# daultanigaurav/AI-BASED-FRAME-INTERPOLATION

Hardware: AMD Instinct MI355X
Metric: interpolated frames/sec at 1080p (higher is better)
Workload: dtype bf16

## Files before the change

ai_based_frame_interpolation_amd/csrc/conv3x3_kwave.hip.h:

```cpp
#pragma once
#include "conv3x3_mfma.hip.h"

namespace fiunet {

struct KWaveTile {
    static constexpr int BN = 64, TH = 2, TW = 32;
    static constexpr int TWP = 40, THP = TH + 2;
    static constexpr int IN_BYTES = THP * TWP * 64;
    static constexpr int W_BYTES = 3 * BN * 64;
    static constexpr int W_SLOTS = 2;
    static constexpr int WAVE_BYTES = IN_BYTES + W_SLOTS * W_BYTES;
    static constexpr int LDS_BYTES = 4 * WAVE_BYTES;
    static_assert(LDS_BYTES <= 160 * 1024, "one workgroup per CU: 160 KiB of LDS");
    static_assert(16 * 1024 <= WAVE_BYTES, "a wave's partial sums (16 KiB) are exchanged through its own region");
};

template <int EPI, bool X2 = false, typename T = __bf16>
__global__ __launch_bounds__(256, 1) void conv3x3_kwave_kernel(const ConvArgs a)
{
    using Tile = KWaveTile;
    constexpr int PL = Elem<T>::PL;
    static_assert(!X2 || std::is_same_v<T, __bf16>, "two-piece operands are bf16");
    constexpr int TWP = Tile::TWP, THP = Tile::THP, TW = Tile::TW, TH = Tile::TH, BN = Tile::BN;
    constexpr int FR = 2, NF = 4, ROWS_W = 2;
    static_assert(EPI == EPI_PLAIN || EPI == EPI_POOL, "plain or pooled epilogue");
    static_assert(conv_wave_frags(64, 8, 32) == NF, "the epilogue is instantiated for the 64 x 64 wave tile");

    extern __shared__ __attribute__((aligned(16))) char smem[];
    const int tid = threadIdx.x;
    const int lane = tid & 63, wave = __builtin_amdgcn_readfirstlane(tid >> 6);
    const int l15 = lane & 15, lc = lane >> 4;
    char* const my = smem + wave * Tile::WAVE_BYTES;
    char* const lds_in = my;
    char* const lds_w = my + Tile::IN_BYTES;
    const unsigned lds_in_addr = lds_addr_of(lds_in);
    const unsigned lds_w_addr = lds_addr_of(lds_w);

    const ConvTileId id = conv_tile_decode(a, conv_block_remap());
    const int ct = id.ct, b = id.b;
    const int y0 = id.ty * TH, x0 = id.tx * TW;
    const int aH = a.H, aW = a.W;

    const int nplanes = (a.C0 + a.C1) / PL;
    const int p0 = a.C0 / PL;
    const int pbeg = wave * nplanes / 4, pend = (wave + 1) * nplanes / 4;
    constexpr int VP = X2 ? 3 : 1;
    const int nsteps = (pend - pbeg) * 3 * VP;
    f32x4 acc[4][NF];
#pragma unroll
    for (int m = 0; m < 4; ++m) {
        f32x4 v = f32x4{0.f, 0.f, 0.f, 0.f};
        if (wave == 0) {
            const float4 sh = *reinterpret_cast<const float4*>(a.shift + ct * BN + conv_cout_ofs<T>(m, lc));
            v = f32x4{sh.x, sh.y, sh.z, sh.w};
        }
#pragma unroll
        for (int n = 0; n < NF; ++n) acc[m][n] = v;
    }

    const int a_off = l15 * 64 + ((lc ^ swz(l15)) << 4);
    int b_off[3];
#pragma unroll
    for (int kx = 0; kx < 3; ++kx) b_off[kx] = (kx + l15) * 64 + ((lc ^ swz(kx + l15)) << 4);

    const char* const wbase = (const char*)a.wgt + (size_t)ct * BN * 64;
    const unsigned w_lane_off = (unsigned)((lane >> 2) * 64 + (((lane & 3) ^ swz(lane >> 2)) << 4));
    constexpr int NWP = Tile::W_BYTES / 1024;
    auto issue_w = [&](int step) __attribute__((always_inline)) {
        const int lp = step / 3, kx = step - lp * 3;
        int pl = pbeg + lp;
        if constexpr (X2) {
            const int real = pbeg + lp / 3;
            pl = lp % 3 == 1 ? nplanes + real : real;
        }
        const char* wsrc = wbase + ((size_t)(pl * 9 + kx * 3) * a.Cout) * 64;
        const unsigned dst = __builtin_amdgcn_readfirstlane(lds_w_addr + (unsigned)((step & 1) * Tile::W_BYTES));
#pragma unroll
        for (int j = 0; j < NWP; ++j) {
            const int r0 = j * 16, tap = r0 / BN;
            glds16s(wsrc + (size_t)(tap * (a.Cout - BN) + r0) * 64, w_lane_off, dst + j * 1024);
        }
    };
    if (nsteps > 0) issue_w(0);

    constexpr int NPIECE = THP * TWP / 16;
    static_assert(THP * TWP % 16 == 0, "in-tile must be a whole number of 1-KiB pieces");
    const char* const dma_src = (const char*)a.src0 + (size_t)b * aH * aW * a.C0 * sizeof(T) * (X2 ? 2 : 1);
    const char* const dma_src1 = a.C1 > 0 ? (const char*)a.src1 + (size_t)b * aH * aW * a.C1 * sizeof(T) * (X2 ? 2 : 1) : nullptr;
    const unsigned plane_bytes = (unsigned)(aH * aW) * 64u;
    unsigned in_off[NPIECE];
#pragma unroll
    for (int j = 0; j < NPIECE; ++j) {
        const int row = j * 16 + (lane >> 2);
        const int py = row / TWP, px = row - py * TWP;
        const int y = y0 - 1 + py, x = x0 - 1 + px;
        const bool ok = (px < TW + 2) & ((unsigned)y < (unsigned)aH) & ((unsigned)x < (unsigned)aW);
        in_off[j] = ok ? (unsigned)(y * aW + x) * 64u + (((lane & 3) ^ swz(row)) << 4) : ~0u;
        if (!ok) *reinterpret_cast<uint4*>(lds_in + j * 1024 + lane * 16) = make_uint4(0u, 0u, 0u, 0u);
    }
    auto gather_plane = [&](int plane, bool lo) __attribute__((always_inline)) {
        const char* base = plane >= p0 ? dma_src1 + (size_t)(plane - p0 + (lo ? nplanes - p0 : 0)) * plane_bytes
                                       : dma_src + (size_t)(plane + (lo ? p0 : 0)) * plane_bytes;
#pragma unroll
        for (int j = 0; j < NPIECE; ++j)
            if (in_off[j] != ~0u) glds16s(base, in_off[j], __builtin_amdgcn_readfirstlane(lds_in_addr + (unsigned)j * 1024u));
    };
    if (nsteps > 0) gather_plane(pbeg, false);
    lds_dma_wait_all();

    int step = 0;
    const int nvp = (pend - pbeg) * VP;
    for (int vp = 0; vp < nvp; ++vp) {
        const int nreal = pbeg + (vp + 1) / VP, nj = (vp + 1) % VP;
        const bool gather_next = vp + 1 < nvp && !(X2 && nj == 1);
#pragma unroll
        for (int kx = 0; kx < 3; ++kx, ++step) {
            if (step + 1 < nsteps) issue_w(step + 1);
            const char* wcur = lds_w + (step & 1) * Tile::W_BYTES + a_off;
            const bool next_tile = kx == 2 && gather_next;
            uint4 xb[ROWS_W + 2][FR];
            auto load_row = [&](int i) __attribute__((always_inline)) {
#pragma unroll
                for (int f = 0; f < FR; ++f)
                    xb[i][f] = *reinterpret_cast<const uint4*>(lds_in + b_off[kx] + (i * TWP + f * 16) * 64);
            };
#pragma unroll
            for (int i = 0; i < ROWS_W; ++i) load_row(i);
#pragma unroll
            for (int ky = 0; ky < 3; ++ky) {
                uint4 wa[4];
#pragma unroll
                for (int m = 0; m < 4; ++m) wa[m] = *reinterpret_cast<const uint4*>(wcur + (ky * BN + m * 16) * 64);
                if (ky < 2) load_row(ROWS_W + ky);
                if (ky == 1 && next_tile) {
                    asm volatile("s_waitcnt lgkmcnt(0)" ::: "memory");
                    gather_plane(nreal, X2 && nj == 2);
                }
#pragma unroll
                for (int m = 0; m < 4; ++m)
#pragma unroll
                    for (int n = 0; n < NF; ++n) mma_chunk<T>(acc[m][n], wa[m], xb[n / FR + ky][n % FR]);
            }
            lds_dma_wait_all();
        }
    }

    if (wave != 0) {
        float4* o = reinterpret_cast<float4*>(my) + lane;
#pragma unroll
        for (int m = 0; m < 4; ++m)
#pragma unroll
            for (int n = 0; n < NF; ++n)
                o[(m * NF + n) * 64] = make_float4(acc[m][n][0], acc[m][n][1], acc[m][n][2], acc[m][n][3]);
    }
    __syncthreads();
    if (wave != 0) return;
#pragma unroll
    for (int w = 1; w < 4; ++w) {
        const float4* p = reinterpret_cast<const float4*>(smem + w * Tile::WAVE_BYTES) + lane;
#pragma unroll
        for (int m = 0; m < 4; ++m)
#pragma unroll
            for (int n = 0; n < NF; ++n) {
                const float4 q = p[(m * NF + n) * 64];
                acc[m][n][0] += q.x; acc[m][n][1] += q.y; acc[m][n][2] += q.z; acc[m][n][3] += q.w;
            }
    }
    conv_epilogue<T, 64, 8, 32, EPI, X2>(a, acc, b, y0, x0, ct, 0, 0, 0, l15, lc);
}

}
```

ai_based_frame_interpolation_amd/csrc/conv3x3_mfma.hip.h:

```cpp
#pragma once
#include <hip/hip_runtime.h>
#include <stdint.h>
#include <type_traits>

namespace fiunet {

typedef __attribute__((ext_vector_type(4))) float f32x4;
typedef __attribute__((ext_vector_type(8))) __bf16 bf16x8;
typedef __attribute__((ext_vector_type(8))) _Float16 f16x8;

enum SrcMode { SRC_DIRECT = 0, SRC_POOL = 1 , SRC_CONCAT_UP = 2,
               SRC_STEM = 3 ,
               SRC_DIRECT_X2 = 4,
               SRC_STEM_X2 = 5 };
constexpr bool src_is_stem(int mode) { return mode == SRC_STEM || mode == SRC_STEM_X2; }
constexpr bool src_is_x2(int mode) { return mode == SRC_DIRECT_X2 || mode == SRC_STEM_X2; }

__device__ __forceinline__ size_t blk_off(int plane, int y, int x, int H, int W)
{
    return (((size_t)plane * H + y) * W + x) * 64;
}

struct ConvArgs {
    const void* src0;
// ... 411 lines not shown
}

template <typename T, int BN, int TH, int TW, int EPI>
__device__ __forceinline__ void conv_acc_init(const ConvArgs& a, f32x4 (&acc)[4][conv_wave_frags(BN, TH, TW)],
                                              int ct, int wc, int lc)
{
    constexpr int NF = conv_wave_frags(BN, TH, TW);
#pragma unroll
    for (int m = 0; m < 4; ++m) {
        f32x4 v = f32x4{0.f, 0.f, 0.f, 0.f};
        if constexpr (!epi_is_splitk(EPI)) {
            const float4 sh = *reinterpret_cast<const float4*>(a.shift + ct * BN + wc * 64 + conv_cout_ofs<T>(m, lc));
            v = f32x4{sh.x, sh.y, sh.z, sh.w};
        }
#pragma unroll
        for (int n = 0; n < NF; ++n) acc[m][n] = v;
    }
}

__device__ __forceinline__ unsigned relu_pk_bf16(unsigned p) { return pk_max_i16(p, 0u); }
__device__ __forceinline__ void relu_fma(float& sum, float x, float lo, float w)
{
    float t;
    asm("v_max_f32 %1, %3, %2\n\tv_fmac_f32 %0, %1, %4" : "+v"(sum), "=&v"(t) : "v"(x), "v"(lo), "v"(w));
}

template <typename T, int BN, int TH, int TW, int EPI, bool X2 = false>
__device__ __forceinline__ void conv_epilogue(const ConvArgs& a, f32x4 (&acc)[4][conv_wave_frags(BN, TH, TW)],
                                              int b, int y0, int x0, int ct, int split, int wc, int wp,
                                              int l15, int lc)
{
    constexpr int PL = Elem<T>::PL;
    constexpr int FR = TW / 16;
    constexpr int NF = conv_wave_frags(BN, TH, TW);
    constexpr int ROWS_W = NF / FR;
    constexpr int HNC = EPI == EPI_HEAD ? 1 : (EPI == EPI_HEAD3 ? 3 : 0);
    const int aH = a.H, aW = a.W;
    constexpr bool PERM = sizeof(T) == 2;
    const int wbase_c = ct * BN + wc * 64;
    if constexpr (epi_is_splitk(EPI)) {
        const int tile = (((b * a.tilesY) + y0 / TH) * a.tilesX + x0 / TW) * a.nct + ct;
        const int ntile = a.B * a.tilesY * a.tilesX * a.nct;
        const int wave = wp * (BN / 64) + wc;
        float4* o = reinterpret_cast<float4*>(a.kslab) + ((((size_t)split * ntile + tile) * 4 + wave) * (4 * NF)) * 64 + (lc * 16 + l15);
#pragma unroll
        for (int m = 0; m < 4; ++m)
#pragma unroll
            for (int n = 0; n < NF; ++n)
                o[(m * NF + n) * 64] = make_float4(acc[m][n][0], acc[m][n][1], acc[m][n][2], acc[m][n][3]);
        return;
    }
    float hw[HNC > 0 ? HNC : 1][4][4];
#pragma unroll
    for (int c = 0; c < HNC; ++c)
#pragma unroll
        for (int m = 0; m < 4; ++m) {
            const float4 v = *reinterpret_cast<const float4*>(a.head_w + c * 64 + conv_cout_ofs<T>(m, lc));
            hw[c][m][0] = v.x; hw[c][m][1] = v.y; hw[c][m][2] = v.z; hw[c][m][3] = v.w;
        }
    const size_t plane_stride = (size_t)aH * aW * 64;
    const int plane0 = wbase_c / PL;
    const int rec_byte = lc * 16;
    char* const out_img = a.dst ? (char*)a.dst + (size_t)b * plane_stride * (a.Cout / PL) +
                                  (size_t)plane0 * plane_stride + rec_byte : nullptr;
    const int pH = aH >> 1, pW = aW >> 1;
    const size_t pplane_stride = (size_t)pH * pW * 64;
    char* const pool_img = EPI == EPI_POOL ? (char*)a.pool_dst + (size_t)b * pplane_stride * (a.Cout / PL) +
                                             (size_t)plane0 * pplane_stride + rec_byte : nullptr;
    if constexpr (HNC > 0) {
        static_assert(HNC == 0 || NF == 8 || NF == 4, "head reduction is written for 8 or 4 fragments per wave");
        const float floor_v = a.relu ? 0.f : -__builtin_inff();
        float hb[HNC];
#pragma unroll
        for (int c = 0; c < HNC; ++c) hb[c] = a.head_b[c];
        const int nb = ((lc & 1) ? 4 : 0) + ((lc & 2) ? 2 : 0);
#pragma unroll
        for (int c = 0; c < HNC; ++c) {
            float hs[NF];
#pragma unroll
            for (int n = 0; n < NF; ++n) {
                float sum = 0.f;
#pragma unroll
                for (int m = 0; m < 4; ++m)
#pragma unroll
                    for (int j = 0; j < 4; ++j) relu_fma(sum, acc[m][n][j], floor_v, hw[c][m][j]);
                hs[n] = sum;
            }
            if constexpr (NF == 4) {
                float full[NF];
#pragma unroll
                for (int n = 0; n < NF; ++n) {
                    const float p = hs[n] + __shfl_xor(hs[n], 16);
                    full[n] = p + __shfl_xor(p, 32);
                }
                const float mine = lc == 0 ? full[0] : (lc == 1 ? full[1] : (lc == 2 ? full[2] : full[3]));
                const int n = lc;
                const int y = y0 + wp * ROWS_W + n / FR;
                const int x = x0 + (n % FR) * 16 + l15;
                if (y < aH && x < aW) {
                    const size_t o = (size_t)b * a.head_img_stride + ((size_t)c * aH + y) * aW + x;
                    if (a.head_out_u8) a.head_out_u8[o] = postprocess_u8_value(mine + hb[c]);
                    else a.head_out[o] = mine + hb[c];
                }
            } else {
                float t[4], u[2];
#pragma unroll
                for (int i = 0; i < 4; ++i) {
                    const auto r = __builtin_amdgcn_permlane16_swap(__float_as_uint(hs[i]), __float_as_uint(hs[(i + 4) % NF]), false, false);
                    t[i] = __uint_as_float(r[0]) + __uint_as_float(r[1]);
                }
#pragma unroll
                for (int j = 0; j < 2; ++j) {
                    const auto r = __builtin_amdgcn_permlane32_swap(__float_as_uint(t[j]), __float_as_uint(t[j + 2]), false, false);
                    u[j] = __uint_as_float(r[0]) + __uint_as_float(r[1]);
                }
#pragma unroll
                for (int j = 0; j < 2; ++j) {
                    const int n = nb + j;
                    const int y = y0 + wp * ROWS_W + n / FR;
                    const int x = x0 + (n % FR) * 16 + l15;
                    if (y < aH && x < aW) {
                        const size_t o = (size_t)b * a.head_img_stride + ((size_t)c * aH + y) * aW + x;
                        if (a.head_out_u8) a.head_out_u8[o] = postprocess_u8_value(u[j] + hb[c]);
                        else a.head_out[o] = u[j] + hb[c];
                    }
                }
            }
        }
    }
    if constexpr (X2) {
        static_assert(std::is_same_v<T, __bf16>, "the two-piece epilogue belongs to the bf16 kernels");
        if (HNC > 0 && !a.dst) return;
        const size_t ps = (size_t)aH * aW * 64;
        const int npo = a.Cout / 32;
        const size_t blk = (size_t)npo * ps;
        char* const img = (char*)a.dst + (size_t)b * 2 * blk + (size_t)(wbase_c / 32) * ps + lc * 16;
        const int pH2 = aH >> 1, pW2 = aW >> 1;
        const size_t pps = (size_t)pH2 * pW2 * 64, pblk = (size_t)npo * pps;
        char* const pimg = EPI == EPI_POOL ? (char*)a.pool_dst + (size_t)b * 2 * pblk + (size_t)(wbase_c / 32) * pps + lc * 16
                                           : nullptr;
        auto put = [&](char* o, size_t block_bytes, const float (&v)[8]) __attribute__((always_inline)) {
            unsigned h[4], l[4];
#pragma unroll
            for (int i = 0; i < 4; ++i) {
                h[i] = pack_bf16x2_pk(v[2 * i], v[2 * i + 1]);
                l[i] = pack_bf16x2_pk(v[2 * i] - __uint_as_float(h[i] << 16), v[2 * i + 1] - __uint_as_float(h[i] & 0xffff0000u));
            }
            *reinterpret_cast<uint4*>(o) = make_uint4(h[0], h[1], h[2], h[3]);
            *reinterpret_cast<uint4*>(o + block_bytes) = make_uint4(l[0], l[1], l[2], l[3]);
        };
#pragma unroll
        for (int n = 0; n < NF; ++n) {
            const int y = y0 + wp * ROWS_W + n / FR;
            const int x = x0 + (n % FR) * 16 + l15;
            if (y < aH && x < aW) {
#pragma unroll
                for (int g = 0; g < 2; ++g) {
                    float v[8];
#pragma unroll
                    for (int j = 0; j < 4; ++j) {
                        v[j] = a.relu ? fmaxf(acc[2 * g][n][j], 0.f) : acc[2 * g][n][j];
                        v[4 + j] = a.relu ? fmaxf(acc[2 * g + 1][n][j], 0.f) : acc[2 * g + 1][n][j];
                    }
                    put(img + (size_t)(y * aW + x) * 64 + g * ps, blk, v);
                }
            }
        }
        if constexpr (EPI == EPI_POOL) {
#pragma unroll
            for (int n = 0; n < NF; ++n) {
                if (((n / FR) & 1) != 0) continue;
                const int y = y0 + wp * ROWS_W + n / FR;
                const int x = x0 + (n % FR) * 16 + l15;
                const int py = y >> 1, px = x >> 1;
                const bool okp = (py < pH2) && (px < pW2) && ((l15 & 1) == 0);
#pragma unroll
                for (int g = 0; g < 2; ++g) {
                    float v[8];
#pragma unroll
                    for (int h = 0; h < 2; ++h)
#pragma unroll
                        for (int j = 0; j < 4; ++j) {
                            const float cm = fmaxf(acc[2 * g + h][n][j], acc[2 * g + h][n + FR][j]);
                            float r = fmaxf(cm, __uint_as_float(dpp_swap_pairs(__float_as_uint(cm))));
                            if (a.relu) r = fmaxf(r, 0.f);
                            v[4 * h + j] = r;
                        }
                    if (okp) put(pimg + (size_t)(min(py, pH2 - 1) * pW2 + min(px, pW2 - 1)) * 64 + g * pps, pblk, v);
                }
            }
        }
        return;
    }
    if constexpr (EPI == EPI_POOL && PERM) {
#pragma unroll
        for (int n = 0; n < NF; ++n) {
            if (((n / FR) & 1) != 0) continue;
            uint4 pk[2][2];
#pragma unroll
            for (int r = 0; r < 2; ++r) {
                const int nn = n + r * FR;
                const int y = y0 + wp * ROWS_W + nn / FR;
                const int x = x0 + (nn % FR) * 16 + l15;
                const bool ok = (y < aH) && (x < aW);
                char* o = out_img + (size_t)(y * aW + x) * 64;
#pragma unroll
                for (int g = 0; g < 2; ++g) {
                    uint4 v = make_uint4(pack2_pk<T>(acc[2 * g][nn][0], acc[2 * g][nn][1]),
                                         pack2_pk<T>(acc[2 * g][nn][2], acc[2 * g][nn][3]),
                                         pack2_pk<T>(acc[2 * g + 1][nn][0], acc[2 * g + 1][nn][1]),
                                         pack2_pk<T>(acc[2 * g + 1][nn][2], acc[2 * g + 1][nn][3]));
                    if (a.relu) v = make_uint4(relu_pk_bf16(v.x), relu_pk_bf16(v.y), relu_pk_bf16(v.z), relu_pk_bf16(v.w));
                    pk[r][g] = v;
                    if (ok && out_img) *reinterpret_cast<uint4*>(o + g * plane_stride) = v;
                }
            }
            const int y = y0 + wp * ROWS_W + n / FR;
            const int x = x0 + (n % FR) * 16 + l15;
            const int py = y >> 1, px = x >> 1;
            const bool okp = (py < pH) && (px < pW) && ((l15 & 1) == 0);
            char* o = pool_img + (size_t)(min(py, pH - 1) * pW + min(px, pW - 1)) * 64;
#pragma unroll
            for (int g = 0; g < 2; ++g) {
                const uint4 t = pk[0][g], u = pk[1][g];
                const unsigned c0 = pk_max_i16(t.x, u.x), c1 = pk_max_i16(t.y, u.y);
                const unsigned c2 = pk_max_i16(t.z, u.z), c3 = pk_max_i16(t.w, u.w);
                const uint4 m = make_uint4(pk_max_i16(c0, dpp_swap_pairs(c0)), pk_max_i16(c1, dpp_swap_pairs(c1)),
                                           pk_max_i16(c2, dpp_swap_pairs(c2)), pk_max_i16(c3, dpp_swap_pairs(c3)));
                if (okp) *reinterpret_cast<uint4*>(o + g * pplane_stride) = m;
            }
        }
        return;
    }
#pragma unroll
    for (int n = 0; n < NF; ++n) {
        const int y = y0 + wp * ROWS_W + n / FR;
        const int x = x0 + (n % FR) * 16 + l15;
        const bool ok = (y < aH) && (x < aW);
        if (ok && out_img) {
            char* o = out_img + (size_t)(y * aW + x) * 64;
            if constexpr (PERM) {
#pragma unroll
                for (int g = 0; g < 2; ++g) {
                    uint4 pk = make_uint4(pack2<T>(acc[2 * g][n][0], acc[2 * g][n][1]),
                                          pack2<T>(acc[2 * g][n][2], acc[2 * g][n][3]),
                                          pack2<T>(acc[2 * g + 1][n][0], acc[2 * g + 1][n][1]),
                                          pack2<T>(acc[2 * g + 1][n][2], acc[2 * g + 1][n][3]));
                    if (a.relu) pk = make_uint4(relu_pk_bf16(pk.x), relu_pk_bf16(pk.y), relu_pk_bf16(pk.z), relu_pk_bf16(pk.w));
                    *reinterpret_cast<uint4*>(o + g * plane_stride) = pk;
                }
            } else {
#pragma unroll
                for (int m = 0; m < 4; ++m) {
                    float4 v = make_float4(acc[m][n][0], acc[m][n][1], acc[m][n][2], acc[m][n][3]);
                    if (a.relu) v = make_float4(fmaxf(v.x, 0.f), fmaxf(v.y, 0.f), fmaxf(v.z, 0.f), fmaxf(v.w, 0.f));
                    *reinterpret_cast<float4*>(o + m * plane_stride) = v;
                }
            }
        }
    }
    if (EPI == EPI_POOL) {
#pragma unroll
        for (int n = 0; n < NF; ++n) {
            if (((n / FR) & 1) != 0) continue;
            const int y = y0 + wp * ROWS_W + n / FR;
            const int x = x0 + (n % FR) * 16 + l15;
            const int py = y >> 1, px = x >> 1;
            const bool okp = (py < pH) && (px < pW) && ((l15 & 1) == 0);
            char* o = pool_img + (size_t)(min(py, pH - 1) * pW + min(px, pW - 1)) * 64;
            if constexpr (!PERM) {
#pragma unroll
                for (int m = 0; m < 4; ++m) {
                    float r[4];
#pragma unroll
                    for (int j = 0; j < 4; ++j) {
                        const float cm = fmaxf(acc[m][n][j], acc[m][n + FR][j]);
                        r[j] = fmaxf(cm, __uint_as_float(dpp_swap_pairs(__float_as_uint(cm))));
                        if (a.relu) r[j] = fmaxf(r[j], 0.f);
                    }
                    if (okp) *reinterpret_cast<float4*>(o + m * pplane_stride) = make_float4(r[0], r[1], r[2], r[3]);
                }
            } else {
#pragma unroll
                for (int g = 0; g < 2; ++g) {
                    unsigned r[4];
#pragma unroll
                    for (int h = 0; h < 2; ++h) {
                        const int m = 2 * g + h;
                        const unsigned a0 = pk_max_i16(pack2_pk<T>(acc[m][n][0], acc[m][n][1]),
                                                       pack2_pk<T>(acc[m][n + FR][0], acc[m][n + FR][1]));
                        const unsigned a1 = pk_max_i16(pack2_pk<T>(acc[m][n][2], acc[m][n][3]),
                                                       pack2_pk<T>(acc[m][n + FR][2], acc[m][n + FR][3]));
                        r[2 * h] = pk_max_i16(a0, dpp_swap_pairs(a0));
                        r[2 * h + 1] = pk_max_i16(a1, dpp_swap_pairs(a1));
                        if (a.relu) { r[2 * h] = relu_pk_bf16(r[2 * h]); r[2 * h + 1] = relu_pk_bf16(r[2 * h + 1]); }
                    }
                    if (okp) *reinterpret_cast<uint4*>(o + g * pplane_stride) = make_uint4(r[0], r[1], r[2], r[3]);
                }
            }
        }
    }
}

template <typename T, int BN, int TH, int TW, int MODE, int EPI>
__global__ __launch_bounds__(256, conv_occupancy(BN, TH, TW, ConvTile<BN, TH, TW, MODE>::LDS_BYTES)) void conv3x3_mfma_kernel(const ConvArgs a)
{
    using Tile = ConvTile<BN, TH, TW, MODE>;
    constexpr int PL = Elem<T>::PL;
    constexpr int TWP = Tile::TWP, THP = Tile::THP;
    constexpr int WAVES_C = BN / 64, WAVES_P = 4 / WAVES_C;
    constexpr int FR = TW / 16;
    constexpr int NF = conv_wave_frags(BN, TH, TW);
    constexpr int ROWS_W = NF / FR;
    static_assert(NF == 8 || NF == 4, "wave tile must be 64 couts x 128 or 64 pixels");
    static_assert(TH == ROWS_W * WAVES_P && ROWS_W * FR == NF, "tile does not split over the waves");
    static_assert(EPI != EPI_POOL || ROWS_W % 2 == 0, "pooled epilogue: a wave owns whole row pairs");
    static_assert(Tile::LDS_BYTES * conv_occupancy(BN, TH, TW, Tile::LDS_BYTES) <= 160 * 1024, "LDS per CU");
    constexpr int HNC = EPI == EPI_HEAD ? 1 : (EPI == EPI_HEAD3 ? 3 : 0);
    static_assert(HNC == 0 || BN == 64, "fused head needs all 64 couts in one wave");
    static_assert(MODE == SRC_DIRECT || MODE == SRC_CONCAT_UP || MODE == SRC_STEM || MODE == SRC_DIRECT_X2 ||
                  MODE == SRC_STEM_X2, "pooling is fused into the producer");
    constexpr bool X2 = src_is_x2(MODE);
    constexpr bool STEM = src_is_stem(MODE);
    constexpr bool DIRECT = MODE == SRC_DIRECT || MODE == SRC_DIRECT_X2;
    static_assert(!X2 || std::is_same_v<T, __bf16>, "two-piece operands are bf16");
    static_assert(!STEM || (sizeof(T) == 2 && BN == 64), "fused stem: 2-byte output (bf16 / fp16), 64 couts");

    extern __shared__ __attribute__((aligned(16))) char smem[];
    char* const lds_in = smem;
    char* const lds_w = smem + Tile::IN_BYTES;
    const unsigned lds_in_addr = lds_addr_of(lds_in);
    const unsigned lds_w_addr = lds_addr_of(lds_w);

    int lid = conv_block_remap();
    const int ksplit = epi_is_splitk(EPI) ? a.ksplit : 1;
    const int split = lid % ksplit;
    lid /= ksplit;
    const ConvTileId id = conv_tile_decode(a, lid);
    const int ct = id.ct, b = id.b;
    const int y0 = id.ty * TH, x0 = id.tx * TW;

    const int tid = threadIdx.x;
    const int lane = tid & 63, wave = __builtin_amdgcn_readfirstlane(tid >> 6);
    const int l15 = lane & 15, lc = lane >> 4;
    const int wc = wave % WAVES_C, wp = wave / WAVES_C;

#ifdef FIUNET_STAMP
    unsigned long long st_sum[16] = {0, 0, 0, 0, 0, 0, 0, 0, 0, 0, 0, 0, 0, 0, 0, 0};
    unsigned long long st_t0 = __builtin_amdgcn_s_memtime(), st_prev = st_t0;
#ifdef FIUNET_STAMP_PROLOG
    unsigned long long st_pprev = st_t0;
#define PSTAMP(slot) do { __builtin_amdgcn_sched_barrier(0); const unsigned long long t_ = __builtin_amdgcn_s_memtime(); \
                          st_sum[slot] += t_ - st_pprev; st_pprev = t_; __builtin_amdgcn_sched_barrier(0); } while (0)
#else
#define PSTAMP(slot) do {} while (0)
#endif
#define STAMP(slot) do { const unsigned long long t_ = __builtin_amdgcn_s_memtime(); \
                         st_sum[slot] += t_ - st_prev; st_prev = t_; } while (0)
#define STAMP_UP(slot) STAMP(slot)
#else
#define STAMP(slot) do {} while (0)
#define STAMP_UP(slot) do {} while (0)
#define PSTAMP(slot) do {} while (0)
#endif
    f32x4 acc[4][NF];
    conv_acc_init<T, BN, TH, TW, EPI>(a, acc, ct, wc, lc);
#ifdef FIUNET_STAMP_PROLOG
    asm volatile("" :: "v"(acc[3][NF - 1][3]), "v"(acc[0][0][0]));
#endif
    PSTAMP(9);

    const int a_off = (wc * 64 + l15) * 64 + ((lc ^ swz(l15)) << 4);
    int b_off[3];
#pragma unroll
    for (int kx = 0; kx < 3; ++kx)
        b_off[kx] = (wp * ROWS_W * TWP + kx + l15) * 64 + ((lc ^ swz(kx + l15)) << 4);

    const int nplanes_real = (a.C0 + a.C1) / PL;
    const int nplanes_all = X2 ? 3 * nplanes_real : nplanes_real;
    const int p0 = a.C0 / PL;
    const int pbeg = split * nplanes_all / ksplit, pend = (split + 1) * nplanes_all / ksplit;
    const int nsteps = (pend - pbeg) * 3;
    const char* wbase = (const char*)a.wgt + (size_t)ct * BN * 64;

    constexpr int NW = Tile::W_BYTES / 1024 / 4;
    static_assert(BN % 16 == 0, "a weight piece must not straddle two taps");
    const unsigned w_lane_off = (unsigned)((lane >> 2) * 64 + (((lane & 3) ^ swz(lane >> 2)) << 4));
    auto issue_w = [&](int step) __attribute__((always_inline)) {
        const int lp = step / 3, kx = step - lp * 3;
        int pl = pbeg + lp;
        if constexpr (X2) {
            const int real = pl / 3;
            pl = pl - real * 3 == 1 ? nplanes_real + real : real;
        }
        const char* wsrc = wbase + ((size_t)(pl * 9 + kx * 3) * a.Cout) * 64;
        const unsigned dst = __builtin_amdgcn_readfirstlane(
            lds_w_addr + (unsigned)((step & 1) * Tile::W_STRIDE + wave * NW * 1024));
#pragma unroll
        for (int j = 0; j < NW; ++j) {
            const int r0 = (wave * NW + j) * 16, tap = r0 / BN;
            glds16s(wsrc + (size_t)(tap * (a.Cout - BN) + r0) * 64, w_lane_off, dst + j * 1024);
        }
    };
#ifndef FIUNET_DIAG_FREE_PROLOGUE
    issue_w(0);
#endif
#ifdef FIUNET_DIAG_NO_WSTREAM
    if (nsteps > 1) issue_w(1);
#endif
    PSTAMP(10);

    constexpr int NPIECE = THP * TWP / 16;
    static_assert(THP * TWP % 16 == 0, "in-tile must be a whole number of 1-KiB pieces");
    const int aH = a.H, aW = a.W;
    const char* const dma_src = (const char*)a.src0 + (size_t)b * a.H * a.W * a.C0 * sizeof(T) * (X2 ? 2 : 1);
    const char* const dma_src1 = DIRECT && a.C1 > 0
                                     ? (const char*)a.src1 + (size_t)b * a.H * a.W * a.C1 * sizeof(T) * (X2 ? 2 : 1) : nullptr;
    constexpr bool HOIST = (MODE == SRC_DIRECT && BN == 128 && EPI == EPI_PLAIN) ||
                           (NF == 4 && DIRECT);
    constexpr bool ROLL = sizeof(T) == 2 && FR == 2 && (!epi_is_splitk(EPI) || NF == 4);
    constexpr int NPW = (NPIECE + 3) / 4;
    unsigned in_off[HOIST ? NPW : 1];
    const unsigned plane_bytes = (unsigned)(aH * aW) * 64u;
    unsigned pm_lin0 = 0, pm_valid = 0, pm_wrap = 0;
    static_assert(NPW <= 32, "one mask bit per piece of a wave");
    constexpr int PM_DY = 64 / TWP, PM_DX = 64 % TWP;
    const unsigned pm_dlin = (unsigned)(PM_DY * aW + PM_DX) * 64u, pm_dwrap = (unsigned)(aW - TWP) * 64u;
    if constexpr (!STEM) {
        const int row0 = wave * 16 + (lane >> 2);
        int py = row0 / TWP, px = row0 - py * TWP;
        int y = y0 - 1 + py, x = x0 - 1 + px;
        pm_lin0 = (unsigned)(y * aW + x) * 64u + (((lane & 3) ^ swz(row0)) << 4);
        unsigned lin = pm_lin0;
#pragma unroll
        for (int jj = 0; jj < NPW; ++jj) {
            const bool ok = (px < TW + 2) & ((unsigned)y < (unsigned)aH) & ((unsigned)x < (unsigned)aW);
            if constexpr (HOIST) in_off[jj] = ok ? lin : ~0u;
            pm_valid |= (ok ? 1u : 0u) << jj;
            px += PM_DX; x += PM_DX; y += PM_DY;
            lin += pm_dlin;
            if (px >= TWP) { px -= TWP; x -= TWP; y += 1; pm_wrap |= 1u << jj; lin += pm_dwrap; }
        }
    }
    auto for_pieces = [&](auto&& f) __attribute__((always_inline)) {
        if constexpr (HOIST) {
#pragma unroll
            for (int jj = 0; jj < NPW; ++jj) {
                const int j = wave + 4 * jj;
                if (j < NPIECE) f(j, in_off[jj] != ~0u, in_off[jj]);
            }
        } else {
            unsigned lin = pm_lin0, valid = pm_valid, wrap = pm_wrap;
            asm volatile("" : "+v"(lin), "+v"(valid), "+v"(wrap));
#pragma unroll
            for (int jj = 0; jj < NPW; ++jj) {
                const int j = wave + 4 * jj;
                if (j < NPIECE) f(j, ((valid >> jj) & 1u) != 0u, lin);
                lin += pm_dlin + (((wrap >> jj) & 1u) ? pm_dwrap : 0u);
            }
        }
    };
    if constexpr (!STEM) {
        for_pieces([&](int j, bool ok, unsigned) __attribute__((always_inline)) {
            if (!ok) *reinterpret_cast<uint4*>(lds_in + j * 1024 + lane * 16) = make_uint4(0u, 0u, 0u, 0u);
        });
    }
    auto gather_plane_dma = [&](int plane) __attribute__((always_inline)) {
        const char* base;
        if constexpr (X2) {
            const int real = plane / 3, lo = plane - real * 3 == 2;
            base = real >= p0 ? dma_src1 + (size_t)(real - p0 + (lo ? nplanes_real - p0 : 0)) * plane_bytes
                              : dma_src + (size_t)(real + (lo ? p0 : 0)) * plane_bytes;
        } else {
            base = (MODE == SRC_DIRECT && plane >= p0) ? dma_src1 + (size_t)(plane - p0) * plane_bytes
                                                       : dma_src + (size_t)plane * plane_bytes;
        }
        for_pieces([&](int j, bool ok, unsigned off) __attribute__((always_inline)) {
            if (ok) glds16s(base, off, __builtin_amdgcn_readfirstlane(lds_in_addr + (unsigned)j * 1024u));
        });
    };

    constexpr int UP_NCOL = (TW + 2) * 4;
    constexpr int UP_NMAIN = UP_NCOL / 64;
    constexpr int UP_NTC = UP_NCOL - UP_NMAIN * 64;
    constexpr int UP_WPG = 4 / UP_NMAIN;
    constexpr int UP_SEGR = (THP + UP_WPG - 1) / UP_WPG;
    constexpr int UP_NTAIL = UP_NTC * THP;
    constexpr int UP_TAILW = (UP_NTAIL + 3) / 4;
    static_assert(MODE != SRC_CONCAT_UP || (UP_NMAIN >= 1 && UP_NMAIN <= 2), "interpolation work split");
    int lr_y = 0, lr_x = 0;
    char* const ytab = smem + Tile::TAB_OFF;
    char* const xtab = ytab + THP * 16;
    uint4 yrow = make_uint4(0u, 0u, 0u, 0u);
    if constexpr (MODE == SRC_CONCAT_UP) {
        const UpCoord u = up_coord(a, y0 - 1, x0 - 1);
        lr_y = u.y0; lr_x = u.x0;
        {
            const int y = y0 - 1 + min(lane, THP - 1);
            const UpAxis uy = up_axis_y(a, min(max(y, 0), a.H - 1));
            const bool ok = uy.ok & (y >= 0) & (y < a.H);
            yrow = make_uint4(ok ? (unsigned)((uy.i0 - lr_y) * (Tile::LRP * 64)) : 0x80000000u,
                              (unsigned)((uy.i1 - lr_y) * (Tile::LRP * 64)), __float_as_uint(uy.h),
                              __float_as_uint(uy.l));
            if (tid < THP) *reinterpret_cast<uint4*>(ytab + tid * 16) = yrow;
        }
        if (tid >= 64 && tid < 64 + TW + 2) {
            const int px = tid - 64, x = x0 - 1 + px;
            const UpAxis ux = up_axis_x(a, min(max(x, 0), a.W - 1));
            const bool ok = ux.ok & (x >= 0) & (x < a.W);
            *reinterpret_cast<uint4*>(xtab + px * 16) =
                make_uint4(ok ? (unsigned)((ux.i0 - lr_x) * 64) : 0x80000000u, (unsigned)((ux.i1 - lr_x) * 64),
                           __float_as_uint(ux.h), __float_as_uint(ux.l));
        }
    }
    auto gather_plane_up = [&](int plane, int idle_slot) __attribute__((always_inline)) {
        constexpr int LRP = Tile::LRP, LRH = Tile::LRH;
        const int stg_off = idle_slot == 0 ? 0 : Tile::W_BYTES;
        const char* const lsrc = (const char*)a.src1 + (size_t)b * a.lowH * a.lowW * a.C1 * sizeof(T) +
                                 (size_t)(plane - p0) * a.lowH * a.lowW * 64;
        int opq = 0;
        asm volatile("" : "+s"(opq));
        int l4 = (lane & 3) << 4;
        asm volatile("" : "+v"(l4));
#pragma unroll 1
        for (int j = wave; j < Tile::LR_PIECES; j += 4) {
            const int row = j * 16 + (lane >> 2) + opq;
            const int r = row / LRP, c = row - r * LRP;
            const int gy = min(lr_y + min(r, LRH - 1), a.lowH - 1), gx = min(lr_x + c, a.lowW - 1);
            const char* src = lsrc + ((unsigned)(gy * a.lowW + gx) * 64u + (unsigned)l4);
            glds16(src, __builtin_amdgcn_readfirstlane(lds_w_addr + (unsigned)(stg_off + j * 1024)));
        }
        lds_dma_wait_all();
        __syncthreads();
        STAMP_UP(6);
        const char* const stg = lds_w + stg_off;
        constexpr int NE = Elem<T>::NE;
        {
            const int grp = UP_NMAIN == 1 ? 0 : (wave & 1), seg = UP_NMAIN == 1 ? wave : (wave >> 1);
            const int col = grp * 64 + lane, px = col >> 2, ch = col & 3;
            const uint4 xt = *reinterpret_cast<const uint4*>(xtab + px * 16);
            const bool okx = (int)xt.x >= 0;
            const char* const s0 = stg + (okx ? (int)xt.x : 0) + ch * 16;
            const char* const s1 = stg + (okx ? (int)xt.y : 0) + ch * 16;
            const float hx = okx ? __uint_as_float(xt.z) : 0.f, lx = okx ? __uint_as_float(xt.w) : 0.f;
            float h0[NE], h1[NE];
#pragma unroll
            for (int i = 0; i < NE; ++i) h0[i] = h1[i] = 0.f;
            int c0 = -1, c1 = -1;
            const int rbeg = seg * UP_SEGR, rend = min(THP, rbeg + UP_SEGR);
#pragma unroll 1
            for (int py = rbeg; py < rend; ++py) {
                const uint4 yt = make_uint4((unsigned)__builtin_amdgcn_readlane((int)yrow.x, py),
                                            (unsigned)__builtin_amdgcn_readlane((int)yrow.y, py),
                                            (unsigned)__builtin_amdgcn_readlane((int)yrow.z, py),
                                            (unsigned)__builtin_amdgcn_readlane((int)yrow.w, py));
                const int o0 = (int)yt.x, o1 = (int)yt.y;
                uint4 v = make_uint4(0u, 0u, 0u, 0u);
                if (o0 >= 0) {
                    if (o0 != c0) {
                        if (o0 == c1) {
#pragma unroll
                            for (int i = 0; i < NE; ++i) h0[i] = h1[i];
                        } else {
                            chunk_hlerp<T>(*reinterpret_cast<const uint4*>(s0 + o0),
                                           *reinterpret_cast<const uint4*>(s1 + o0), hx, lx, h0);
                        }
                        c0 = o0;
                    }
                    if (o1 != c1) {
                        if (o1 == c0) {
#pragma unroll
                            for (int i = 0; i < NE; ++i) h1[i] = h0[i];
                        } else {
                            chunk_hlerp<T>(*reinterpret_cast<const uint4*>(s0 + o1),
                                           *reinterpret_cast<const uint4*>(s1 + o1), hx, lx, h1);
                        }
                        c1 = o1;
                    }
                    v = chunk_vlerp<T>(h0, h1, __uint_as_float(yt.z), __uint_as_float(yt.w));
                }
                const int row = py * TWP + px;
                *reinterpret_cast<uint4*>(lds_in + row * 64 + ((ch ^ swz(row)) << 4)) = v;
            }
        }
        for (int k = lane; k < UP_TAILW; k += 64) {
            const int e = wave * UP_TAILW + k;
            if (e < UP_NTAIL) {
                const int py = e / UP_NTC, col = UP_NMAIN * 64 + (e - py * UP_NTC), px = col >> 2, ch = col & 3;
                const uint4 xt = *reinterpret_cast<const uint4*>(xtab + px * 16);
                const uint4 yt = *reinterpret_cast<const uint4*>(ytab + py * 16);
                const bool ok = ((int)xt.x >= 0) & ((int)yt.x >= 0);
                const char* const q0 = stg + (ok ? (int)xt.x : 0) + ch * 16;
                const char* const q1 = stg + (ok ? (int)xt.y : 0) + ch * 16;
                const int o0 = ok ? (int)yt.x : 0, o1 = ok ? (int)yt.y : 0;
                uint4 v = chunk_bilerp<T>(*reinterpret_cast<const uint4*>(q0 + o0), *reinterpret_cast<const uint4*>(q1 + o0),
                                          *reinterpret_cast<const uint4*>(q0 + o1), *reinterpret_cast<const uint4*>(q1 + o1),
                                          __uint_as_float(xt.z), __uint_as_float(xt.w), __uint_as_float(yt.z),
                                          __uint_as_float(yt.w));
                if (!ok) v = make_uint4(0u, 0u, 0u, 0u);
                const int row = py * TWP + px;
                *reinterpret_cast<uint4*>(lds_in + row * 64 + ((ch ^ swz(row)) << 4)) = v;
            }
        }
        STAMP_UP(7);
    };

    constexpr int NIN = THP * (TW + 2);
    char* const patch = smem + Tile::PATCH_OFF;
    constexpr int PW = Tile::PATCH_W, PH = Tile::PATCH_H, PP = Tile::PATCH_PITCH;
    auto stage_patch = [&]() __attribute__((always_inline)) {
        if constexpr (STEM) {
            unsigned* const pd = reinterpret_cast<unsigned*>(patch);
            constexpr int NP = PH * PW;
            constexpr int NB = (NP + 255) / 256;
            float v0[NB], v1[NB];
            unsigned okm = 0;
            size_t at[NB];
#pragma unroll
            for (int k = 0; k < NB; ++k) {
                const int r = tid + k * 256;
                const int py = r / PW, px = r - py * PW;
                const int y = y0 - 2 + py, x = x0 - 2 + px;
                const bool ok = (r < NP) & (y >= 0) & (y < aH) & (x >= 0) & (x < aW);
                okm |= (ok ? 1u : 0u) << k;
                at[k] = ((size_t)b * aH + min(max(y, 0), aH - 1)) * aW + min(max(x, 0), aW - 1);
            }
            if (a.u1) {
                unsigned char q0[NB], q1[NB];
#pragma unroll
                for (int k = 0; k < NB; ++k) { q0[k] = a.u1[at[k]]; q1[k] = a.u2[at[k]]; }
#pragma unroll
                for (int k = 0; k < NB; ++k) { v0[k] = preprocess_u8_value(q0[k]); v1[k] = preprocess_u8_value(q1[k]); }
            } else {
#pragma unroll
                for (int k = 0; k < NB; ++k) { v0[k] = a.f1[at[k]]; v1[k] = a.f2[at[k]]; }
            }
#pragma unroll
            for (int k = 0; k < NB; ++k) {
                const int r = tid + k * 256;
                const int py = r / PW, px = r - py * PW;
                const float d = a.dither * stem_dither(y0 - 2 + py, x0 - 2 + px);
                const bool ok = (okm >> k) & 1u;
                v0[k] = ok ? v0[k] + d : 0.f;
                v1[k] = ok ? v1[k] - d : 0.f;
            }
#pragma unroll
            for (int k = 0; k < NB; ++k) {
                const int r = tid + k * 256;
                const int py = r / PW, px = r - py * PW;
                const unsigned hi = pack_bf16x2_pk(v0[k], v1[k]);
                const unsigned lo = pack_bf16x2_pk(v0[k] - __uint_as_float(hi << 16), v1[k] - __uint_as_float(hi & 0xffff0000u));
                if (r < NP) {
                    pd[py * PP + px] = hi;
                    pd[py * PP + px + PW] = lo;
                }
            }
            if (tid < 2 * PW) reinterpret_cast<unsigned*>(smem + Tile::PATCH_TAIL_OFF)[tid] = tid < PW ? 0x00003f80u : 0u;
        }
    };
    struct StemW { uint4 wh[2], wl[2]; };
    StemW stem_w0;
    auto stem_park = [&](int plane) __attribute__((always_inline)) {
        if constexpr (STEM && X2)
            glds16s((const char*)a.stem_w + (wave >> 1) * 4096 + (2 * plane + (wave & 1)) * 1024, (unsigned)lane * 16u,
                    __builtin_amdgcn_readfirstlane(lds_in_addr + (unsigned)(Tile::STEMW_OFF + wave * 1024)));
        else if constexpr (STEM)
            glds16((const char*)a.stem_w + (wave >> 1) * 4096 + (2 * plane + (wave & 1)) * 1024 + lane * 16,
                   __builtin_amdgcn_readfirstlane(lds_in_addr + (unsigned)(Tile::STEMW_OFF + wave * 1024)));
    };
    auto stem_load = [&](StemW& w) __attribute__((always_inline)) {
        if constexpr (STEM) {
            int lane_ofs = l15 * 64 + lc * 16;
            asm volatile("" : "+v"(lane_ofs));
#pragma unroll
            for (int h = 0; h < 2; ++h) {
                w.wh[h] = ldg16((const char*)a.stem_w + h * 1024 + lane_ofs);
                w.wl[h] = ldg16((const char*)a.stem_w + 4096 + h * 1024 + lane_ofs);
            }
            stem_park(X2 ? 0 : 1);
        }
    };
    auto stem_parked = [&](StemW& w) __attribute__((always_inline)) {
        if constexpr (STEM) {
            const char* const base = smem + Tile::STEMW_OFF + l15 * 64 + lc * 16;
#pragma unroll
            for (int h = 0; h < 2; ++h) {
                w.wh[h] = *reinterpret_cast<const uint4*>(base + h * 1024);
                w.wl[h] = *reinterpret_cast<const uint4*>(base + 2048 + h * 1024);
            }
        }
    };
    auto gather_plane_stem = [&](const StemW& w, bool lo_piece = false) __attribute__((always_inline)) {
        if constexpr (STEM) {
            constexpr int TAIL_IDX = (Tile::PATCH_TAIL_OFF - Tile::PATCH_OFF) / 4;
            const unsigned* const ph32 = reinterpret_cast<const unsigned*>(patch);
            const unsigned* const pl32 = ph32 + PW;
            struct Frag { uint4 bh, bl; int dst; };
            constexpr int DY = 64 / (TW + 2), DX = 64 % (TW + 2);
            const int py0 = (wave * 16 + l15) / (TW + 2);
            int px = wave * 16 + l15 - py0 * (TW + 2);
            int e = lc < 3 ? py0 * PP + px + (lc == 0 ? 0 : (lc == 1 ? 2 * PP : PP)) : TAIL_IDX;
            const int e_step = lc < 3 ? DY * PP + DX : 0, e_wrap = lc < 3 ? PP - (TW + 2) : 0;
            int dst = py0 * TWP + px;
            auto fetch = [&](Frag& f) __attribute__((always_inline)) {
                f.bh = make_uint4(ph32[e], ph32[e + 1], ph32[e + 2], ph32[e + 3]);
                f.bl = make_uint4(pl32[e], pl32[e + 1], pl32[e + 2], pl32[e + 3]);
                f.dst = dst;
                px += DX;
                const bool wrap = px >= TW + 2;
                px -= wrap ? TW + 2 : 0;
                e += e_step + (wrap ? e_wrap : 0);
                dst += DY * TWP + DX + (wrap ? TWP - (TW + 2) : 0);
            };
            auto compute = [&](const Frag& f) __attribute__((always_inline)) {
                f32x4 s4[2];
#pragma unroll
                for (int h = 0; h < 2; ++h) s4[h] = f32x4{0.f, 0.f, 0.f, 0.f};
#pragma unroll
                for (int h = 0; h < 2; ++h) mma_chunk<__bf16>(s4[h], w.wl[h], f.bh);
#pragma unroll
                for (int h = 0; h < 2; ++h) mma_chunk<__bf16>(s4[h], w.wh[h], f.bl);
#pragma unroll
                for (int h = 0; h < 2; ++h) mma_chunk<__bf16>(s4[h], w.wh[h], f.bh);
                const int row = f.dst;
                uint4 pk = make_uint4(relu_pk_bf16(pack2_pk<T>(s4[0][0], s4[0][1])),
                                      relu_pk_bf16(pack2_pk<T>(s4[0][2], s4[0][3])),
                                      relu_pk_bf16(pack2_pk<T>(s4[1][0], s4[1][1])),
                                      relu_pk_bf16(pack2_pk<T>(s4[1][2], s4[1][3])));
                if constexpr (X2) {
                    if (lo_piece) {
                        auto lo2 = [](float v0, float v1, unsigned hi) __attribute__((always_inline)) {
                            return pack_bf16x2_pk(fmaxf(v0, 0.f) - __uint_as_float(hi << 16),
                                                  fmaxf(v1, 0.f) - __uint_as_float(hi & 0xffff0000u));
                        };
                        pk = make_uint4(lo2(s4[0][0], s4[0][1], pk.x), lo2(s4[0][2], s4[0][3], pk.y),
                                        lo2(s4[1][0], s4[1][1], pk.z), lo2(s4[1][2], s4[1][3], pk.w));
                    }
                }
                if (row < THP * TWP) *reinterpret_cast<uint4*>(lds_in + ((row * 64 + lc * 16) ^ ((row & 4) << 3))) = pk;
            };
            constexpr int NQ = (NIN + 15) / 16;
            Frag fa, fb;
            fetch(fa);
#pragma unroll 1
            for (int q = wave; q < NQ; q += 8) {
                fetch(fb);
                compute(fa);
                fetch(fa);
                if (q + 4 < NQ) compute(fb);
            }
            if ((y0 == 0) | (x0 == 0) | (y0 + TH >= aH) | (x0 + TW >= aW)) {
                __syncthreads();
                for (int i = tid; i < THP * (TW + 2) * 4; i += 256) {
                    const int q = i >> 2, ch = i & 3;
                    const int qy = q / (TW + 2), qx = q - qy * (TW + 2);
                    const bool in = ((unsigned)(y0 - 1 + qy) < (unsigned)aH) & ((unsigned)(x0 - 1 + qx) < (unsigned)aW);
                    const int row = qy * TWP + qx;
                    if (!in) *reinterpret_cast<uint4*>(lds_in + row * 64 + ((ch ^ swz(row)) << 4)) = make_uint4(0u, 0u, 0u, 0u);
                }
            }
        }
    };
    auto gather_plane = [&](int plane, int idle_slot, bool first) __attribute__((always_inline)) {
        if constexpr (STEM && X2) {
            if (first) {
                gather_plane_stem(stem_w0, false);
            } else {
                StemW w;
                stem_parked(w);
                gather_plane_stem(w, plane == 2 || plane == 5);
            }
        } else if constexpr (STEM) {
            if (first) {
                gather_plane_stem(stem_w0);
            } else {
                StemW w1;
                stem_parked(w1);
                gather_plane_stem(w1);
            }
        }
        else if (DIRECT || plane < p0) gather_plane_dma(plane);
        else gather_plane_up(plane, idle_slot);
    };

    PSTAMP(11);
    if constexpr (STEM) {
        stem_load(stem_w0);
        stage_patch();
        __syncthreads();
        PSTAMP(12);
    }
#ifdef FIUNET_DIAG_FREE_PROLOGUE
    if constexpr (STEM || MODE == SRC_CONCAT_UP) gather_plane(pbeg, 1, true);
#else
    gather_plane(pbeg, 1, true);
#endif
    PSTAMP(13);
    lds_dma_wait_all();
    PSTAMP(14);
    __syncthreads();
    PSTAMP(15);
    STAMP(1);
#ifdef FIUNET_CLOCK
    const unsigned long long ck_t0 = __builtin_amdgcn_s_memtime(), ck_r0 = __builtin_amdgcn_s_memrealtime();
#endif

    int step = 0;
    int vj = X2 ? pbeg % 3 : 0;
    for (int plane = pbeg; plane < pend; ++plane) {
        const bool gather_next = plane + 1 < pend && !(X2 && vj == 0);
        if constexpr (X2) vj = vj == 2 ? 0 : vj + 1;
#pragma unroll
        for (int kx = 0; kx < 3; ++kx, ++step) {
#ifndef FIUNET_DIAG_NO_WSTREAM
            if (step + 1 < nsteps) issue_w(step + 1);
#endif
            const char* wcur = lds_w + (step & 1) * Tile::W_STRIDE + a_off;
            constexpr bool EARLY_OK = ROLL && DIRECT;
            bool early = false;
            if constexpr (EARLY_OK)
                early = kx == 2 && gather_next && (DIRECT || plane + 1 < p0);
            if constexpr (ROLL) {
                uint4 xb[ROWS_W + 2][FR];
                auto load_row = [&](int i) __attribute__((always_inline)) {
#pragma unroll
                    for (int f = 0; f < FR; ++f)
                        xb[i][f] = *reinterpret_cast<const uint4*>(lds_in + b_off[kx] + (i * TWP + f * 16) * 64);
                };
#pragma unroll
                for (int i = 0; i < ROWS_W; ++i) load_row(i);
#pragma unroll
                for (int ky = 0; ky < 3; ++ky) {
                    uint4 wa[4];
#pragma unroll
                    for (int m = 0; m < 4; ++m)
                        wa[m] = *reinterpret_cast<const uint4*>(wcur + (ky * BN + m * 16) * 64);
                    if (ky < 2) load_row(ROWS_W + ky);
                    if (ky == 1 && early) {
                        __syncthreads();
                        gather_plane(plane + 1, step & 1, false);
                    }
#pragma unroll
                    for (int m = 0; m < 4; ++m)
#pragma unroll
                        for (int n = 0; n < NF; ++n) mma_chunk<T>(acc[m][n], wa[m], xb[n / FR + ky][n % FR]);
                }
            } else {
#pragma unroll
                for (int ky = 0; ky < 3; ++ky) {
                    asm volatile("" ::: "memory");
                    uint4 wa[4], xb[NF];
#pragma unroll
                    for (int m = 0; m < 4; ++m)
                        wa[m] = *reinterpret_cast<const uint4*>(wcur + (ky * BN + m * 16) * 64);
#pragma unroll
                    for (int n = 0; n < NF; ++n)
                        xb[n] = *reinterpret_cast<const uint4*>(
                            lds_in + b_off[kx] + (((n / FR) + ky) * TWP + (n % FR) * 16) * 64);
#pragma unroll
                    for (int m = 0; m < 4; ++m)
#pragma unroll
                        for (int n = 0; n < NF; ++n) mma_chunk<T>(acc[m][n], wa[m], xb[n]);
                }
            }
#ifdef FIUNET_STAMP
            asm volatile("" :: "v"(acc[3][NF - 1][3]));
            __builtin_amdgcn_sched_barrier(0);
#endif
            STAMP(2);
            if (kx == 2 && gather_next && !early) {
                __syncthreads();
                gather_plane(plane + 1, step & 1, false);
                lds_dma_wait_all();
                __syncthreads();
                if constexpr (STEM && X2) { if (plane + 1 == 2) stem_park(1); }
                STAMP(4);
            } else {
                lds_dma_wait_all();
                __syncthreads();
                STAMP(3);
            }
        }
    }

#ifdef FIUNET_CLOCK
    {
        asm volatile("" :: "v"(acc[3][NF - 1][3]));
        __builtin_amdgcn_sched_barrier(0);
        const unsigned long long ck_t1 = __builtin_amdgcn_s_memtime(), ck_r1 = __builtin_amdgcn_s_memrealtime();
        const unsigned st_idx = blockIdx.x * 4u + (unsigned)wave;
        if (a.stamp && lane == 0 && st_idx < a.stamp_cap) {
            unsigned long long* rec = a.stamp + (size_t)st_idx * 16;
            rec[0] = ck_t1 - ck_t0;
            rec[1] = ck_r1 - ck_r0;
            rec[8] = 1ull;
        }
    }
#endif
    conv_epilogue<T, BN, TH, TW, EPI, X2>(a, acc, b, y0, x0, ct, split, wc, wp, l15, lc);
#ifdef FIUNET_STAMP
    STAMP(5);
    st_sum[0] = st_prev - st_t0;
    const unsigned st_idx = blockIdx.x * 4u + (unsigned)wave;
    if (a.stamp && lane == 0 && st_idx < a.stamp_cap) {
        unsigned long long* rec = a.stamp + (size_t)st_idx * 16;
#pragma unroll
        for (int k = 0; k < 16; ++k) rec[k] = k == 8 ? 1ull : st_sum[k];
    }
#endif
}

template <typename T, int BN, int TH, int TW, int EPI, bool X2>
__global__ __launch_bounds__(64) void splitk_finalize_tile_kernel(const ConvArgs a)
{
    static_assert(EPI == EPI_PLAIN || EPI == EPI_POOL, "a fused head is never K-split");
    constexpr int WAVES_C = BN / 64;
    constexpr int NF = conv_wave_frags(BN, TH, TW);
    int t = blockIdx.x >> 2;
    const int tile = t;
    const int ct = t % a.nct; t /= a.nct;
    const int tx = t % a.tilesX; t /= a.tilesX;
    const int ty = t % a.tilesY;
    const int b = t / a.tilesY;
    const int lane = threadIdx.x & 63, wave = blockIdx.x & 3;
    const int l15 = lane & 15, lc = lane >> 4;
    const int wc = wave % WAVES_C, wp = wave / WAVES_C;
    const int ntile = a.B * a.tilesY * a.tilesX * a.nct;
    f32x4 acc[4][NF];
#pragma unroll
    for (int m = 0; m < 4; ++m)
#pragma unroll
        for (int n = 0; n < NF; ++n) acc[m][n] = f32x4{0.f, 0.f, 0.f, 0.f};
    const float4* p = reinterpret_cast<const float4*>(a.kslab) + (((size_t)tile * 4 + wave) * (4 * NF)) * 64 + lane;
    const size_t slice = (size_t)ntile * 4 * (4 * NF) * 64;
    const int ks = a.ksplit;
#pragma unroll
    for (int m = 0; m < 4; ++m) {
        const float4* pm = p + (size_t)m * NF * 64;
        constexpr int CH = NF == 8 ? 2 : 4;
        for (int s0 = 0; s0 < ks; s0 += CH, pm += CH * slice) {
            float4 q[CH][NF];
#pragma unroll
            for (int j = 0; j < CH; ++j)
                if (s0 + j < ks) {
#pragma unroll
                    for (int n = 0; n < NF; ++n) q[j][n] = pm[j * slice + n * 64];
                }
#pragma unroll
            for (int j = 0; j < CH; ++j)
                if (s0 + j < ks) {
#pragma unroll
                    for (int n = 0; n < NF; ++n) {
                        acc[m][n][0] += q[j][n].x; acc[m][n][1] += q[j][n].y; acc[m][n][2] += q[j][n].z; acc[m][n][3] += q[j][n].w;
                    }
                }
        }
    }
#pragma unroll
    for (int m = 0; m < 4; ++m) {
        const float4 sh = *reinterpret_cast<const float4*>(a.shift + ct * BN + wc * 64 + conv_cout_ofs<T>(m, lc));
#pragma unroll
        for (int n = 0; n < NF; ++n) {
            acc[m][n][0] += sh.x; acc[m][n][1] += sh.y; acc[m][n][2] += sh.z; acc[m][n][3] += sh.w;
        }
    }
    conv_epilogue<T, BN, TH, TW, EPI, X2>(a, acc, b, ty * TH, tx * TW, ct, 0, wc, wp, l15, lc);
}

}
```

Baseline: 533.6.

## Move K-loop barrier and weight prefetch into mid-step rendezvous in MFMA conv

For selected bf16 conv tile shapes, the per-step barrier and the weight-slice DMA issue move from the step boundary to a rendezvous placed between MFMA blocks. Weights are prefetched two steps ahead, and the next input plane's gather overlaps the remaining MFMAs. The aim is to hide barrier and DMA latency behind tensor work. This raises register and schedule complexity and depends on correct wait counts. It also adds an lgkmcnt wait at the top of each step in the k-wave kernel.

```diff
diff --git a/ai_based_frame_interpolation_amd/csrc/conv3x3_kwave.hip.h b/ai_based_frame_interpolation_amd/csrc/conv3x3_kwave.hip.h
--- a/ai_based_frame_interpolation_amd/csrc/conv3x3_kwave.hip.h
+++ b/ai_based_frame_interpolation_amd/csrc/conv3x3_kwave.hip.h
@@ -115,6 +115,7 @@
         const bool gather_next = vp + 1 < nvp && !(X2 && nj == 1);
 #pragma unroll
         for (int kx = 0; kx < 3; ++kx, ++step) {
+            asm volatile("s_waitcnt lgkmcnt(0)" ::: "memory");
             if (step + 1 < nsteps) issue_w(step + 1);
             const char* wcur = lds_w + (step & 1) * Tile::W_BYTES + a_off;
             const bool next_tile = kx == 2 && gather_next;
diff --git a/ai_based_frame_interpolation_amd/csrc/conv3x3_mfma.hip.h b/ai_based_frame_interpolation_amd/csrc/conv3x3_mfma.hip.h
--- a/ai_based_frame_interpolation_amd/csrc/conv3x3_mfma.hip.h
+++ b/ai_based_frame_interpolation_amd/csrc/conv3x3_mfma.hip.h
@@ -737,6 +737,27 @@
     }
 }
 
+#if defined(FIUNET_MIDSTEP) && !defined(FIUNET_MIDSTEP_SKIP)
+#define FIUNET_MIDSTEP_SKIP 0
+#endif
+constexpr int conv_midstep(bool bf16, int BN, int TH, int TW, int MODE, int EPI)
+{
+#ifdef FIUNET_MIDSTEP
+    return (FIUNET_MIDSTEP) | (FIUNET_MIDSTEP_SKIP) << 3;
+#else
+    if (!bf16 || TW != 32) return 0;
+    if (BN == 128 && TH == 8 && MODE == SRC_DIRECT && (EPI == EPI_PLAIN || EPI == EPI_POOL)) return 3;
+    if (BN == 64 && TH == 16 && MODE == SRC_DIRECT && EPI == EPI_HEAD) return 1 | 1 << 3;
+    return 0;
+#endif
+}
+__device__ __forceinline__ void kloop_rendezvous()
+{
+    __builtin_amdgcn_sched_barrier(0);
+    asm volatile("s_waitcnt vmcnt(0) lgkmcnt(0)\n\ts_barrier" ::: "memory");
+    __builtin_amdgcn_sched_barrier(0);
+}
+
 template <typename T, int BN, int TH, int TW, int MODE, int EPI>
 __global__ __launch_bounds__(256, conv_occupancy(BN, TH, TW, ConvTile<BN, TH, TW, MODE>::LDS_BYTES)) void conv3x3_mfma_kernel(const ConvArgs a)
 {
@@ -761,6 +782,11 @@
     static_assert(!X2 || std::is_same_v<T, __bf16>, "two-piece operands are bf16");
     static_assert(!STEM || (sizeof(T) == 2 && BN == 64), "fused stem: 2-byte output (bf16 / fp16), 64 couts");
 
+    constexpr bool ROLL = sizeof(T) == 2 && FR == 2 && (!epi_is_splitk(EPI) || NF == 4);
+    constexpr int MID = ROLL ? conv_midstep(std::is_same_v<T, __bf16>, BN, TH, TW, MODE, EPI) & 7 : 0;
+    constexpr int MSKIP = conv_midstep(std::is_same_v<T, __bf16>, BN, TH, TW, MODE, EPI) >> 3;
+    static_assert(MID <= 3 && MSKIP <= 3, "conv_midstep: placement | skipped MFMA blocks << 3");
+
     extern __shared__ __attribute__((aligned(16))) char smem[];
     char* const lds_in = smem;
     char* const lds_w = smem + Tile::IN_BYTES;
@@ -842,6 +868,9 @@
 #endif
 #ifdef FIUNET_DIAG_NO_WSTREAM
     if (nsteps > 1) issue_w(1);
+#else
+    const bool w1_late = MODE == SRC_CONCAT_UP && pbeg >= p0;
+    if constexpr (MID != 0) { if (nsteps > 1 && !w1_late) issue_w(1); }
 #endif
     PSTAMP(10);
 
@@ -853,7 +882,6 @@
                                      ? (const char*)a.src1 + (size_t)b * a.H * a.W * a.C1 * sizeof(T) * (X2 ? 2 : 1) : nullptr;
     constexpr bool HOIST = (MODE == SRC_DIRECT && BN == 128 && EPI == EPI_PLAIN) ||
                            (NF == 4 && DIRECT);
-    constexpr bool ROLL = sizeof(T) == 2 && FR == 2 && (!epi_is_splitk(EPI) || NF == 4);
     constexpr int NPW = (NPIECE + 3) / 4;
     unsigned in_off[HOIST ? NPW : 1];
     const unsigned plane_bytes = (unsigned)(aH * aW) * 64u;
@@ -1234,6 +1262,9 @@
     lds_dma_wait_all();
     PSTAMP(14);
     __syncthreads();
+#ifndef FIUNET_DIAG_NO_WSTREAM
+    if constexpr (MID != 0) { if (nsteps > 1 && w1_late) issue_w(1); }
+#endif
     PSTAMP(15);
     STAMP(1);
 #ifdef FIUNET_CLOCK
@@ -1248,13 +1279,14 @@
 #pragma unroll
         for (int kx = 0; kx < 3; ++kx, ++step) {
 #ifndef FIUNET_DIAG_NO_WSTREAM
-            if (step + 1 < nsteps) issue_w(step + 1);
+            if constexpr (MID == 0) { if (step + 1 < nsteps) issue_w(step + 1); }
 #endif
             const char* wcur = lds_w + (step & 1) * Tile::W_STRIDE + a_off;
             constexpr bool EARLY_OK = ROLL && DIRECT;
             bool early = false;
             if constexpr (EARLY_OK)
                 early = kx == 2 && gather_next && (DIRECT || plane + 1 < p0);
+            const bool up_next = MODE == SRC_CONCAT_UP && kx == 2 && gather_next && plane + 1 >= p0;
             if constexpr (ROLL) {
                 uint4 xb[ROWS_W + 2][FR];
                 auto load_row = [&](int i) __attribute__((always_inline)) {
@@ -1264,21 +1296,49 @@
                 };
 #pragma unroll
                 for (int i = 0; i < ROWS_W; ++i) load_row(i);
+                uint4 wa2[MID == 2 ? 4 : 1];
 #pragma unroll
                 for (int ky = 0; ky < 3; ++ky) {
                     uint4 wa[4];
 #pragma unroll
-                    for (int m = 0; m < 4; ++m)
-                        wa[m] = *reinterpret_cast<const uint4*>(wcur + (ky * BN + m * 16) * 64);
+                    for (int m = 0; m < 4; ++m) {
+                        if (MID == 2 && ky == 2) wa[m] = wa2[m];
+                        else wa[m] = *reinterpret_cast<const uint4*>(wcur + (ky * BN + m * 16) * 64);
+                    }
+                    if constexpr (MID == 2) {
+                        if (ky == 1) {
+#pragma unroll
+                            for (int m = 0; m < 4; ++m)
+                                wa2[m] = *reinterpret_cast<const uint4*>(wcur + (2 * BN + m * 16) * 64);
+                        }
+                    }
                     if (ky < 2) load_row(ROWS_W + ky);
-                    if (ky == 1 && early) {
+                    if (MID == 0 && ky == 1 && early) {
                         __syncthreads();
                         gather_plane(plane + 1, step & 1, false);
                     }
-#pragma unroll
-                    for (int m = 0; m < 4; ++m)
+                    auto rendezvous = [&]() __attribute__((always_inline)) {
+                        if (MID == 3 && ky == 1 && early) {
+                            kloop_rendezvous();
+                            gather_plane(plane + 1, step & 1, false);
+                            __builtin_amdgcn_sched_barrier(0);
+                        }
+                        if (MID != 0 && ky == (MID == 2 ? 1 : 2) && !(MID == 3 && early)) {
+                            kloop_rendezvous();
+#ifndef FIUNET_DIAG_NO_WSTREAM
+                            if (step + 2 < nsteps && !up_next) issue_w(step + 2);
+#endif
+                            if (early) gather_plane(plane + 1, step & 1, false);
+                            __builtin_amdgcn_sched_barrier(0);
+                        }
+                    };
+                    if (MSKIP == 0) rendezvous();
+#pragma unroll
+                    for (int m = 0; m < 4; ++m) {
+                        if (MSKIP != 0 && m == MSKIP) rendezvous();
 #pragma unroll
                         for (int n = 0; n < NF; ++n) mma_chunk<T>(acc[m][n], wa[m], xb[n / FR + ky][n % FR]);
+                    }
                 }
             } else {
 #pragma unroll
@@ -1303,16 +1363,35 @@
             __builtin_amdgcn_sched_barrier(0);
 #endif
             STAMP(2);
-            if (kx == 2 && gather_next && !early) {
+            if constexpr (MID == 0) {
+                if (kx == 2 && gather_next && !early) {
+                    __syncthreads();
+                    gather_plane(plane + 1, step & 1, false);
+                    lds_dma_wait_all();
+                    __syncthreads();
+                    if constexpr (STEM && X2) { if (plane + 1 == 2) stem_park(1); }
+                    STAMP(4);
+                } else {
+#ifdef FIUNET_DIAG_NO_STEP_BARRIER
+                    if (kx == 2)
+#endif
+                    {
+                        lds_dma_wait_all();
+                        __syncthreads();
+                    }
+                    STAMP(3);
+                }
+            } else if (kx == 2 && gather_next) {
+                if (!early) gather_plane(plane + 1, step & 1, false);
+                lds_dma_wait_all();
+                if constexpr (MID == 3) asm volatile("s_waitcnt lgkmcnt(0)" ::: "memory");
                 __syncthreads();
-                gather_plane(plane + 1, step & 1, false);
-                lds_dma_wait_all();
-                __syncthreads();
+#ifndef FIUNET_DIAG_NO_WSTREAM
+                if ((up_next || (MID == 3 && early)) && step + 2 < nsteps) issue_w(step + 2);
+#endif
                 if constexpr (STEM && X2) { if (plane + 1 == 2) stem_park(1); }
                 STAMP(4);
             } else {
-                lds_dma_wait_all();
-                __syncthreads();
                 STAMP(3);
             }
         }
```

After: 537.4 (median of 5 runs). About the same (+0.7%).
